# biddisco/hpx

Hardware: AMD Instinct MI355X
Metric: achieved GB/s (% HBM peak) for triad/reduce/scan/sort at 2^30, 1-8 MI355X (higher is better)
Workload: dtype f64+int64; 1 GPU; STREAM triad (f64) + transform_reduce (int64) + inclusive_scan (int64) per step; elements_per_gpu=1073741824, global_elements=1073741824, partitioning=partitioned_vector x1

## Files before the change

### hpx_amd/_lib.py

```python
from __future__ import annotations

import ctypes
import os
import threading

_HERE = os.path.dirname(os.path.abspath(__file__))
LIB_PATH = os.path.join(_HERE, "libhpxhip.so")

I32, U32, I64, U64, F32, F64 = range(6)
PLUS, MULTIPLIES, MIN, MAX, BIT_AND, BIT_OR, BIT_XOR = range(7)
U_IDENTITY, U_SCALE, U_ADD_SCALAR, U_AFFINE, U_NEGATE, U_ABS, U_SQUARE = range(7)
B_ADD, B_TRIAD, B_SUB, B_MUL, B_AXPY, B_MIN, B_MAX = range(7)
P_LT, P_LE, P_GT, P_GE, P_EQ, P_NE, P_NOT_LT, P_BITS = range(8)
H2H, H2D, D2H, D2D, DEFAULT = range(5)
GEN_IOTA, GEN_BITS, GEN_RANGE, GEN_UNIT = range(4)
(ALGO_REDUCE, ALGO_SCAN, ALGO_COPY_IF, ALGO_SORT, ALGO_SORT_BY_KEY, ALGO_MERGE, ALGO_MERGE_RUNS,
 ALGO_REDUCE_BY_KEY) = range(8)
STENCIL_MAX_FUSED = 16

SUCCESS = 0
ERROR_INVALID_ARGUMENT = 10001
ERROR_UNSUPPORTED = 10002
ERROR_DEVICE_TIMEOUT = 10003
ERROR_OUT_OF_MEMORY = 10004
# ... 84 lines not shown
    "hpxhip_stream_device": [_vp, ctypes.POINTER(_i)],
    "hpxhip_event_destroy": [_vp],
    "hpxhip_event_record": [_vp, _vp],
    "hpxhip_event_synchronize": [_vp],
    "hpxhip_event_query": [_vp],
    "hpxhip_event_elapsed_ms": [_vp, _vp, ctypes.POINTER(_f)],
    "hpxhip_stream_wait_event": [_vp, _vp],
    "hpxhip_malloc": [_i, ctypes.POINTER(_vp), _sz],
    "hpxhip_free": [_vp],
    "hpxhip_malloc_host": [ctypes.POINTER(_vp), _sz],
    "hpxhip_free_host": [_vp],
    "hpxhip_mem_info": [_i, ctypes.POINTER(_sz), ctypes.POINTER(_sz)],
    "hpxhip_memcpy_async": [_vp, _vp, _sz, _i, _vp],
    "hpxhip_memcpy_peer_async": [_vp, _i, _vp, _i, _sz, _vp],
    "hpxhip_memset_async": [_vp, _i, _sz, _vp],
    "hpxhip_scratch_bytes": [_i, _i, _i, _u64, ctypes.POINTER(_sz)],
    "hpxhip_stream_scratch": [_vp, _sz, ctypes.POINTER(_vp)],
    "hpxhip_device_error_word": [_vp, ctypes.POINTER(_vp)],
    "hpxhip_generate": [_i, _i, _u64, ctypes.c_int64, ctypes.c_int64, _vp, _u64, _vp],
    "hpxhip_generate_at": [_i, _i, _u64, _u64, ctypes.c_int64, ctypes.c_int64, _vp, _u64, _vp],
    "hpxhip_fill": [_i, _vp, _vp, _u64, _vp],
    "hpxhip_copy": [_i, _vp, _vp, _u64, _vp],
    "hpxhip_for_each": [_i, _i, _vp, _vp, _u64, _vp],
    "hpxhip_transform": [_i, _i, _i, _i, _vp, _vp, _vp, _u64, _vp],
    "hpxhip_transform_binary": [_i, _i, _i, _i, _vp, _vp, _vp, _vp, _u64, _vp],
    "hpxhip_transform_strided": [_i, _i, _i, _i, _vp, _vp, ctypes.c_int64, _vp, ctypes.c_int64, _u64, _vp],
    "hpxhip_transform_binary_strided": [_i, _i, _i, _i, _vp, _vp, ctypes.c_int64, _vp, ctypes.c_int64, _vp,
                                        ctypes.c_int64, _u64, _vp],
    "hpxhip_transform_reduce": [_i, _i, _i, _i, _vp, _vp, _vp, _u64, _vp, _vp, _vp, _sz],
    "hpxhip_transform_reduce_binary": [_i, _i, _i, _i, _vp, _vp, _vp, _vp, _u64, _vp, _vp, _vp, _sz],
    "hpxhip_fold": [_i, _i, _vp, _vp, _u64, _vp, _vp],
    "hpxhip_fold_exclusive": [_i, _i, _vp, _vp, _u64, _vp, _vp],
    "hpxhip_scan": [_i, _i, _i, _i, _vp, _vp, _vp, _vp, _vp, _u64, _vp, _vp, _sz],
    "hpxhip_copy_if": [_i, _i, _vp, _vp, _vp, _u64, _vp, _vp, _vp, _sz],
    "hpxhip_reduce_by_key": [_i, _i, _i, _vp, _vp, _vp, _vp, _u64, _vp, _vp, _vp, _sz],
    "hpxhip_sort": [_i, _vp, _u64, _i, _vp, _vp, _sz],
    "hpxhip_sort_by_key": [_i, _i, _vp, _vp, _u64, _i, _vp, _vp, _sz],
    "hpxhip_merge": [_i, _vp, _u64, _vp, _u64, _vp, _i, _vp, _vp, _sz],
    "hpxhip_merge_runs": [_i, _vp, _vp, _i, _vp, _i, _vp, _vp, _sz],
    "hpxhip_unsorted_pairs": [_i, _vp, _u64, _i, _vp, _vp],
    "hpxhip_sorted_bounds": [_i, _vp, _u64, _vp, _u64, _i, _i, _vp, _vp],
    "hpxhip_stencil_heat_step": [_vp, _vp, _u64, _vp, _vp, _d, _d, _d, _vp],
    "hpxhip_stencil_heat_run": [_vp, _vp, _u64, _u64, _d, _d, _d, _vp],
    "hpxhip_stencil_heat_steps": [_vp, _vp, _u64, _u64, _u64, _vp, _vp, _i, _d, _d, _d, _vp],
    "hpxhip_stencil_heat_run_fused": [_vp, _vp, _u64, _u64, _d, _d, _d, ctypes.POINTER(_i), _vp],
}

_lib = None
_lock = threading.Lock()


def _preload_torch():
    if os.environ.get("HPXHIP_NO_TORCH"):
        return
    try:
        import torch
    except Exception:
        pass


ABI_VERSION = 1


def load(path: str | None = None):
    global _lib
    with _lock:
# ... 53 lines not shown
```

### hpx_amd/csrc/scan.hip

```cpp
#include <cstdlib>

#include "internal.hpp"
#include <hpxhip/kernels/lookback.hpp>
#include <hpxhip/kernels/reduce_by_key_kernel.hpp>
#include <hpxhip/kernels/scan_kernel.hpp>

using namespace hpxhip;

namespace {

using namespace hpxhip::scan_detail;

constexpr size_t kSlotsOff = 256;

template <typename T, int ROUNDS, int THREADS = kThreads>
uint64_t ntiles_for(uint64_t n) {
    return (n + tile_elems<T, ROUNDS, THREADS>() - 1) / tile_elems<T, ROUNDS, THREADS>();
}

template <typename T, bool ALIGNED>
constexpr int threads_for() {
    return (ALIGNED && (std::is_integral_v<T> || sizeof(T) == 8) && rounds_for<T, ALIGNED>() == 16) ? 512 : kThreads;
}

template <typename T>
size_t carry_off(uint64_t n) {
    return align_up(kSlotsOff + ntiles_for<T, 8>(n) * tile_state<T>::bytes_per_tile(), 256);
}
template <typename T>
size_t scratch_total(uint64_t n) {
    return carry_off<T>(n) + 256;
}

template <typename T, bool INCL, bool ALIGNED, bool SHIFTED = false, typename Conv, typename Op>
int launch_scan(const T* in, T* out, uint64_t n, Conv conv, Op op, T init, const T* prefix_dev, char* ws,
                hipStream_t s) {
    static_assert(ALIGNED || !SHIFTED, "a shifted input needs the vector kernel");
    constexpr int R = rounds_for<T, ALIGNED>();
    constexpr int TH = threads_for<T, ALIGNED>();
    static_assert(tile_elems<T, R, TH>() >= tile_elems<T, 8>(), "scratch is sized for 1024 x 8-round tiles");
    const uint64_t ntiles = ntiles_for<T, R, TH>(n);
    HPXHIP_CHECK(hipMemsetAsync(ws, 0, align_up(kSlotsOff + ntiles * tile_state<T>::bytes_per_tile(), 256), s));
    scan_detail::scan_state<T> st{reinterpret_cast<uint64_t*>(ws + kSlotsOff), device_error_word(s)};
    hipLaunchKernelGGL((k_scan<T, Conv, Op, INCL, ALIGNED, R, TH, true, TH == kThreads ? 1 : 4, false, 1,
                               HPXHIP_TILE_DYN_ID, true, T, std::is_floating_point_v<T> && sizeof(T) == 8, true,
                               SHIFTED>),
                       dim3(static_cast<unsigned>(ntiles)), dim3(TH), 0, s, in, out, n, conv, op, init, prefix_dev,
                       reinterpret_cast<uint32_t*>(ws), st);
    HPXHIP_CHECK_LAUNCH();
    return 0;
}

template <typename T, bool INCL, typename Conv, typename Op>
__global__ void k_scan_head(const T* in, T* out, uint64_t h, Conv conv, Op op, T init, const T* prefix_dev,
                            T* carry) {
    if (threadIdx.x != 0 || blockIdx.x != 0) return;
    T acc = prefix_dev ? *prefix_dev : init;
    for (uint64_t i = 0; i < h; ++i) {
        const T x = conv(in[i]);
        if (INCL) {
            acc = op(acc, x);
            out[i] = acc;
        } else {
            out[i] = acc;
            acc = op(acc, x);
        }
    }
    *carry = acc;
}

template <typename T, bool INCL, typename Conv, typename Op>
int launch_scan_split(const T* in, T* out, uint64_t n, Conv conv, Op op, T init, const T* prefix_dev, char* ws,
                      hipStream_t s) {
    const uintptr_t ia = reinterpret_cast<uintptr_t>(in), oa = reinterpret_cast<uintptr_t>(out);
    if (ia % sizeof(T) != 0 || oa % sizeof(T) != 0) return -1;
    uint64_t h = head_to_align16(out, sizeof(T));
    const uintptr_t v = oa + h * sizeof(T);
    h += ((1024 - v % 1024) % 1024) / sizeof(T);
    if (n <= 4 * h + 1024) return -1;
    T* carry = reinterpret_cast<T*>(ws + carry_off<T>(n));
    hipLaunchKernelGGL((k_scan_head<T, INCL, Conv, Op>), dim3(1), dim3(64), 0, s, in, out, h, conv, op, init,
                       prefix_dev, carry);
    HPXHIP_CHECK_LAUNCH();
    if (ia % 16 == oa % 16) return launch_scan<T, INCL, true>(in + h, out + h, n - h, conv, op, init, carry, ws, s);
    return launch_scan<T, INCL, true, true>(in + h, out + h, n - h, conv, op, init, carry, ws, s);
}

template <typename T, typename F>
int with_scan_conv(int kind, const void* scalars, F&& f) {
    switch (kind) {
        case HPXHIP_U_IDENTITY:
        case HPXHIP_U_SCALE:
        case HPXHIP_U_SQUARE: break;
        default: return HPXHIP_ERROR_UNSUPPORTED;
    }
    return with_unary<T>(kind, scalars, [&](auto conv) -> int {
        using C = decltype(conv);
        if constexpr (std::is_same_v<C, unary_fn<HPXHIP_U_IDENTITY, T>> ||
                      std::is_same_v<C, unary_fn<HPXHIP_U_SCALE, T>> ||
                      std::is_same_v<C, unary_fn<HPXHIP_U_SQUARE, T>>)
            return f(conv);
        else
            return HPXHIP_ERROR_UNSUPPORTED;
    });
}

}

namespace hpxhip {
size_t scan_scratch_bytes(int dtype, uint64_t n) {
    return dtype_size(dtype) == 8 ? scratch_total<uint64_t>(n) : scratch_total<uint32_t>(n);
}
}

namespace {

namespace rbk = hpxhip::reduce_by_key_detail;

// ... 44 lines not shown
    return launch_reduce_by_key_ct<K, V, uint32_t>(kp, vp, ko, vo, n, f, count_dev, base, s);
}

template <typename F>
int with_key_class(int key_dtype, F&& f) {
    switch (key_dtype) {
        case HPXHIP_I32:
        case HPXHIP_U32: return f(tag<uint32_t>{});
        case HPXHIP_I64:
        case HPXHIP_U64: return f(tag<uint64_t>{});
        case HPXHIP_F32: return f(tag<float>{});
        case HPXHIP_F64: return f(tag<double>{});
        default: return HPXHIP_ERROR_INVALID_ARGUMENT;
    }
}

template <typename V, typename F>
int with_value_op(int op, F&& f) {
    if constexpr (std::is_integral_v<V> && std::is_signed_v<V>) {
        switch (op) {
            case HPXHIP_MIN: return f(op_min{});
            case HPXHIP_MAX: return f(op_max{});
            default: return HPXHIP_ERROR_INVALID_ARGUMENT;
        }
    } else {
        return with_binop<V>(op, f);
    }
}

__global__ void k_zero_u64(uint64_t* c) {
    if (threadIdx.x == 0 && blockIdx.x == 0) *c = 0;
}

}

namespace hpxhip {
size_t reduce_by_key_scratch_bytes(int key_dtype, int value_dtype, uint64_t n) {
    (void)key_dtype;
    return dtype_size(value_dtype) == 8 ? rbk_state_bytes<uint64_t, uint64_t>(n, true)
                                        : rbk_state_bytes<uint64_t, uint32_t>(n, true);
}
}

extern "C" int hpxhip_reduce_by_key(int key_dtype, int value_dtype, int op, const void* keys_in,
                                    const void* values_in, void* keys_out, void* values_out, uint64_t n,
                                    uint64_t* count_dev, hpxhip_stream stream, void* scratch, size_t scratch_bytes) {
    HPXHIP_ANNOTATE("hpxhip_reduce_by_key");
    if (!count_dev || (n && (!keys_in || !values_in || !keys_out || !values_out)))
        return HPXHIP_ERROR_INVALID_ARGUMENT;
    if (dtype_size(key_dtype) == 0 || dtype_size(value_dtype) == 0) return HPXHIP_ERROR_INVALID_ARGUMENT;
    if (op < HPXHIP_PLUS || op > HPXHIP_BIT_XOR) return HPXHIP_ERROR_INVALID_ARGUMENT;
    hipStream_t s = reinterpret_cast<hipStream_t>(stream);
    device_guard g(s);
    if (g.status) return g.status;
    if (n == 0) {
        hipLaunchKernelGGL(k_zero_u64, dim3(1), dim3(64), 0, s, count_dev);
        HPXHIP_CHECK_LAUNCH();
        return 0;
    }
    if (op != HPXHIP_MIN && op != HPXHIP_MAX) {
        if (value_dtype == HPXHIP_I32) value_dtype = HPXHIP_U32;
        if (value_dtype == HPXHIP_I64) value_dtype = HPXHIP_U64;
    }
    return with_key_class(key_dtype, [&](auto kt) -> int {
        using K = typename decltype(kt)::type;
        return with_dtype(value_dtype, [&](auto vt) -> int {
            using V = typename decltype(vt)::type;
            return with_value_op<V>(op, [&](auto o) -> int {
                return launch_reduce_by_key<K, V>(keys_in, values_in, keys_out, values_out, n, o, count_dev, s,
                                                  scratch, scratch_bytes);
            });
        });
    });
}

extern "C" int hpxhip_scan(int dtype, int op, int inclusive, int conv_kind, const void* conv_scalars,
                           const void* init, const void* prefix_dev, const void* in, void* out, uint64_t n,
                           hpxhip_stream stream, void* scratch, size_t scratch_bytes) {
    HPXHIP_ANNOTATE("hpxhip_scan");
    if (n == 0) return 0;
    if (!in || !out || (!init && !prefix_dev)) return HPXHIP_ERROR_INVALID_ARGUMENT;
    hipStream_t s = reinterpret_cast<hipStream_t>(stream);
    device_guard g(s);
    if (g.status) return g.status;
    return with_dtype(dtype, [&](auto t) -> int {
        using T = typename decltype(t)::type;
        T iv = T(0);
        if (init) __builtin_memcpy(&iv, init, sizeof(T));
        return with_binop<T>(op, [&](auto o) -> int {
            return with_scan_conv<T>(conv_kind, conv_scalars, [&](auto conv) -> int {
                void* ws = nullptr;
                int rc = resolve_scratch(s, scratch, scratch_bytes, scratch_total<T>(n), &ws);
                if (rc) return rc;
                char* base = static_cast<char*>(ws);
                const bool aligned = (reinterpret_cast<uintptr_t>(in) % 16 == 0) &&
                                     (reinterpret_cast<uintptr_t>(out) % 16 == 0);
                const T* pd = static_cast<const T*>(prefix_dev);
                const T* ip = static_cast<const T*>(in);
                T* op_ = static_cast<T*>(out);
                if (inclusive) {
                    if (aligned) return launch_scan<T, true, true>(ip, op_, n, conv, o, iv, pd, base, s);
                    const int r = launch_scan_split<T, true>(ip, op_, n, conv, o, iv, pd, base, s);
                    return r >= 0 ? r : launch_scan<T, true, false>(ip, op_, n, conv, o, iv, pd, base, s);
                }
                if (aligned) return launch_scan<T, false, true>(ip, op_, n, conv, o, iv, pd, base, s);
                const int r = launch_scan_split<T, false>(ip, op_, n, conv, o, iv, pd, base, s);
                return r >= 0 ? r : launch_scan<T, false, false>(ip, op_, n, conv, o, iv, pd, base, s);
            });
        });
    });
}
```

### hpx_amd/segmented.py

```python
from __future__ import annotations

import contextlib
import ctypes
import os

import numpy as np

from . import _lib as L
from . import functional as F
from .compute import dtype_code, np_dtype, target, vector


def partition_bounds(n: int, parts: int, k: int):
    part = -(-n // parts) if parts else 0
    b = min(n, k * part)
    return b, min(n, b + part)


def rank_partitions(k: int, p: int, r: int):
    c = -(-k // p) if p else 0
    a = min(k, r * c)
    return a, min(k, a + c)


# ... 217 lines not shown
            self.mem.put(h[0:c], send_left, nb, stream)
            self.mem.put(h[M:M + c], send_right, nb, stream)
            for w in dist.batch_isend_irecv(ring_halo_ops(dist, self.rank, self.size, h[0:c], h[M:M + c],
                                                           h[2 * M:2 * M + c], h[3 * M:3 * M + c])):
                w.wait()
            self.mem.get(recv_left, h[2 * M:2 * M + c], nb, stream)
            self.mem.get(recv_right, h[3 * M:3 * M + c], nb, stream)


class HipEngine:

    def __init__(self, tgt: target):
        self.tgt = tgt

    @property
    def stream(self):
        return self.tgt.stream

    def reduce_into(self, vec, lo, hi, op, conv, acc_dt, out_ptr, init=None):
        seed = _identity(op.kind, acc_dt) if init is None else init
        L.call("hpxhip_transform_reduce", vec.dtype, acc_dt, op.kind, conv.kind, L.scalars_buf(acc_dt, conv.scalars),
               L.scalar_buf(acc_dt, seed), ctypes.c_void_p(vec.data() + lo * vec.value_size), hi - lo,
               ctypes.c_void_p(out_ptr), self.stream, None, 0)

    def fold(self, dt, op, init, values_ptr, count, out_ptr):
        L.call("hpxhip_fold", dt, op.kind, L.scalar_buf(dt, init), ctypes.c_void_p(values_ptr), count,
               ctypes.c_void_p(out_ptr), self.stream)

    def scan(self, src, lo, hi, dst, dlo, op, conv, inclusive, prefix_ptr):
        dt = src.dtype
        L.call("hpxhip_scan", dt, op.kind, 1 if inclusive else 0, conv.kind, L.scalars_buf(dt, conv.scalars),
               L.scalar_buf(dt, 0), ctypes.c_void_p(prefix_ptr), ctypes.c_void_p(src.data() + lo * src.value_size),
               ctypes.c_void_p(dst.data() + dlo * dst.value_size), hi - lo, self.stream, None, 0)

    def transform(self, pol, pv, lo, hi, dst, dlo, f):
        from . import algorithms as A
        A.transform((pol or _par()).on(_exec(pv)), pv.local.begin() + lo, pv.local.begin() + hi, dst.begin() + dlo, f)

    def word(self, ptr, i, size=8):
        return ptr + size * int(i)

    def put(self, ptr, dt, value):
        L.call("hpxhip_fill", dt, L.scalar_buf(dt, value), ctypes.c_void_p(ptr), 1, self.stream)

    def read(self, ptr, dt):
        out = np.empty(1, np_dtype(dt))
        L.call("hpxhip_memcpy_async", out.ctypes.data_as(ctypes.c_void_p), ctypes.c_void_p(ptr), out.itemsize, L.D2H,
               self.stream)
        L.call("hpxhip_stream_synchronize", self.stream)
        return out[0].item()

    def sort(self, vec, lo, hi, descending):
        if hi - lo > 1:
            L.call("hpxhip_sort", vec.dtype, ctypes.c_void_p(vec.data() + lo * vec.value_size), hi - lo,
                   1 if descending else 0, self.stream, None, 0)

    def bounds(self, vec, lo, hi, values, upper, descending):
        values = np.ascontiguousarray(values, np_dtype(vec.dtype))
        m = values.size
        dv = vector.from_host(values, self.tgt)
        dout = vector(m, dtype=np.uint64, tgt=self.tgt)
        L.call("hpxhip_sorted_bounds", vec.dtype, ctypes.c_void_p(vec.data() + lo * vec.value_size), hi - lo,
               ctypes.c_void_p(dv.data()), m, 1 if upper else 0, 1 if descending else 0,
               ctypes.c_void_p(dout.data()), self.stream)
        out = dout.to_host()
        dv.free()
# ... 367 lines not shown
                return future.on_stream(eng.stream, thunk=lambda: _read_host(host, adt))
            return make_ready_future(eng.read(dev, adt))
        if isinstance(eng, HipEngine):
            from .algorithms import _read_host
            L.call("hpxhip_memcpy_async", ctypes.c_void_p(hslot), ctypes.c_void_p(dev), 8, L.D2H, eng.stream)
            L.call("hpxhip_stream_synchronize", eng.stream)
            return _read_host(hslot, adt)
        return eng.read(dev, adt)

    def reduce(self, pol, first, last, init=0, op=F.plus):
        return self.transform_reduce(pol, first, last, init, op, F.identity())

    def _scan(self, pol, first, last, dest, op, init, inclusive, conv):
        op = F.require(op, F.BinaryOp, "segmented scan")
        conv = F.require(conv, F.Unary, "segmented scan")
        pv, a, b = _range(first, last)
        pd, d0, _ = _range(dest, dest + (b - a))
        if pd.dtype != pv.dtype:
            raise TypeError("segmented scan: input and output element types must match")
        eng, comm = self.engine(pv), pv.comm
        plan = self._dest_plan(pv, a, b, pd, d0)
        direct, ia, ib, _, _, at = plan
        from .algorithms import _slots_for
        def carry_slot():
            return _slots_for(pv.tgt).next()[0] if isinstance(eng, HipEngine) else eng.scratch()
        lo0 = ia - pv.lo
        out, out0 = (pd.local, at) if direct else (eng.buffer(pd.local, ib - ia), 0)
        if pv.parts == 1:
            carry = carry_slot()
            send, recv = comm.slots(8)
            eng.fold(pv.dtype, op, init, recv, 0, carry)
            if ib > ia:
                eng.scan(pv.local, lo0, ib - pv.lo, out, out0, op, conv, inclusive, carry)
        else:
            recv, cmax = self._segment_totals(pv, a, b, op, conv, pv.dtype, eng, comm)
            j0, j1 = pv.my_segments()
            for i, j in enumerate(range(j0, j1)):
                s0, s1 = pv.segment_bounds(j)
                lo, hi = pv.local_range(max(s0, a), min(s1, b))
                if hi <= lo:
                    continue
                carry = carry_slot()
                eng.fold(pv.dtype, op, init, recv, comm.rank * cmax + i, carry)
                eng.scan(pv.local, lo, hi, out, out0 + (lo - lo0), op, conv, inclusive, carry)
        if not direct:
            self._finish_dest(eng, comm, plan, out, pd)
        return dest + (b - a)

    def inclusive_scan(self, pol, first, last, dest, op=F.plus, init=0):
        return self._scan(pol, first, last, dest, op, init, True, F.identity())

    def exclusive_scan(self, pol, first, last, dest, init, op=F.plus):
        return self._scan(pol, first, last, dest, op, init, False, F.identity())

    def transform_inclusive_scan(self, pol, first, last, dest, op, conv, init=0):
        return self._scan(pol, first, last, dest, op, init, True, conv)

    def transform_exclusive_scan(self, pol, first, last, dest, init, op, conv):
        return self._scan(pol, first, last, dest, op, init, False, conv)

    def sort(self, pol, first, last=None, comp=F.less):
        comp = F.require(comp, F.Compare, "segmented sort")
        pv, a, b = _range(first, last)
        if a != 0 or b != pv.n:
            raise ValueError("segmented sort sorts a whole partitioned_vector")
        eng, comm = self.engine(pv), pv.comm
# ... 270 lines not shown
```

### include/hpx/parallel/algorithms.hpp

```cpp
#pragma once

#include <hpx/compute/hip.hpp>
#include <hpx/compute/hip/concurrent_executor.hpp>
#include <hpx/compute/hip/default_executor.hpp>
#include <hpx/compute/hip/functional.hpp>
#include <hpx/parallel/detail/device_algorithms.hpp>
#include <hpx/parallel/detail/device_closures.hpp>
#include <hpx/parallel/execution.hpp>
#include <hpx/parallel/segmented_fwd.hpp>

#include <algorithm>
#include <array>
#include <cstring>
#include <functional>
#include <iterator>
#include <tuple>
#include <type_traits>
#include <vector>

namespace hpx { namespace parallel {
inline namespace v1 {

namespace detail {
namespace hip = hpx::compute::hip;
// ... 412 lines not shown
    if constexpr (tr::is_binop<Op> && tr::is_unary<Conv>) {
        T s[2] = {};
        tr::unary_t<Conv>::scalars(conv, s);
        check(hpxhip_transform_reduce(dt<TI>, dt<T>, tr::binop_t<Op>::kind, tr::unary_t<Conv>::kind, s, &init, first, n,
                                      out_dev, t.stream(), nullptr, 0),
              "transform_reduce");
    } else {
#if HPX_HAVE_HIP_DEVICE_CLOSURES
        dev::reduce<T, false>(t, first, static_cast<TI const*>(nullptr), n, init, op, conv, out_dev);
#else
        no_device_mapping<Op>("transform_reduce");
#endif
    }
}

template <typename V, typename Op, typename Conv, typename T>
void scan_into(hip::target const& t, V const* first, V* out, uint64_t n, Op const& op, Conv const& conv, T init,
               V const* prefix_dev, bool inclusive) {
    if constexpr (tr::is_binop<Op> && tr::is_unary<Conv>) {
        V s[2] = {};
        tr::unary_t<Conv>::scalars(conv, s);
        V iv = static_cast<V>(init);
        check(hpxhip_scan(dt<V>, tr::binop_t<Op>::kind, inclusive ? 1 : 0, tr::unary_t<Conv>::kind, s, &iv, prefix_dev,
                          first, out, n, t.stream(), nullptr, 0),
              inclusive ? "inclusive_scan" : "exclusive_scan");
    } else {
#if HPX_HAVE_HIP_DEVICE_CLOSURES
        if (prefix_dev)
            throw hpx::exception(HPXHIP_ERROR_UNSUPPORTED, "scan: a device prefix needs a built-in operator");
        dev::scan(t, first, out, n, op, conv, init, inclusive);
#else
        no_device_mapping<Op>(inclusive ? "inclusive_scan" : "exclusive_scan");
#endif
    }
}

template <typename T, typename P, typename It, typename Op, typename Conv>
result_t<P, T> reduce_impl(P&& p, It first, It last, T init, Op&& op, Conv&& conv) {
    if constexpr (is_seg<It>) {
        return segmented_detail::reduce<T>(std::forward<P>(p), first, last, init, std::forward<Op>(op),
                                           std::forward<Conv>(conv));
    } else {
    static_assert(is_dev<It>, "reduce: device iterators required");
    using TI = value_t<It>;
    auto const& t = target_of(p, first);
    auto slot = t.make_result_slot();
    reduce_into<T>(t, static_cast<TI const*>(first.device_ptr()), distance(first, last), init, op, conv, slot.device());
    fetch_slot(t, slot, sizeof(T), "reduce result");
    return finish_slot<T>(p, t, std::move(slot), load_value<T>{});
    }
}
}
namespace algo {

template <typename P, typename It, typename T, typename Op>
detail::result_t<P, T> reduce(P&& p, It first, It last, T init, Op&& op) {
    return detail::reduce_impl<T>(std::forward<P>(p), first, last, init, std::forward<Op>(op),
                                  hpx::compute::hip::functional::identity{});
}
template <typename P, typename It, typename T>
detail::result_t<P, T> reduce(P&& p, It first, It last, T init) {
    return reduce(std::forward<P>(p), first, last, init, std::plus<T>());
}
template <typename P, typename It>
detail::result_t<P, detail::value_t<It>> reduce(P&& p, It first, It last) {
    using T = detail::value_t<It>;
// ... 637 lines not shown
```

### include/hpx/parallel/segmented_algorithms.hpp

```cpp
#pragma once

#include <hpx/parallel/algorithms.hpp>
#include <hpx/parallel/segmented_fwd.hpp>

#include <algorithm>
#include <limits>
#include <vector>

namespace hpx { namespace parallel { inline namespace v1 { namespace segmented_detail {

namespace ex = hpx::parallel::execution;

template <typename P>
constexpr bool task_policy = execution::is_async_execution_policy<typename std::decay<P>::type>::value;

struct segment {
    std::size_t part, lo, hi;
};

template <typename PV>
std::vector<segment> segments_of(PV& pv, std::size_t a, std::size_t b) {
    std::vector<segment> s;
    if (a >= b) return s;
    for (std::size_t j = pv.partition_of(a); j < pv.get_num_partitions(); ++j) {
        auto const& p = pv.get_partition(j);
        if (p.first >= b) break;
        const std::size_t lo = std::max(a, p.first), hi = std::min(b, p.last);
        if (hi > lo) s.push_back(segment{j, lo - p.first, hi - p.first});
    }
    return s;
}

template <typename It>
std::size_t index_of(It const& it) {
    return it.index();
}

template <typename T, typename Op>
// ... 76 lines not shown
    }
    Out end = dest + (last - first);
    return finish<R, P>(std::move(fs), [last, end] { return R{last, end}; });
}

template <typename P, typename In1, typename In2, typename Out, typename F>
typename util::detail::algorithm_result<P, util::tagged_tuple<In1, In2, Out>>::type transform_binary(
    P&&, In1 first1, std::size_t n, In2 first2, Out dest, F&& f) {
    using R = util::tagged_tuple<In1, In2, Out>;
    auto& pv = first1.container();
    auto& p2 = first2.container();
    auto& pd = dest.container();
    require_same_layout(pv, index_of(first1), p2, index_of(first2), "segmented transform");
    require_same_layout(pv, index_of(first1), pd, index_of(dest), "segmented transform");
    using L1 = typename std::decay<decltype(pv.get_partition(0).data->begin())>::type;
    using L2 = typename std::decay<decltype(p2.get_partition(0).data->begin())>::type;
    using LO = typename std::decay<decltype(pd.get_partition(0).data->begin())>::type;
    std::vector<hpx::future<util::tagged_tuple<L1, L2, LO>>> fs;
    const std::size_t a = index_of(first1);
    for (auto const& s : segments_of(pv, a, a + n)) {
        auto& d1 = *pv.get_partition(s.part).data;
        auto& d2 = *p2.get_partition(s.part).data;
        auto& o = *pd.get_partition(s.part).data;
        fs.push_back(hpx::parallel::transform(ex::par(ex::task), d1.begin() + s.lo, d1.begin() + s.hi,
                                              d2.begin() + s.lo, o.begin() + s.lo, f));
    }
    const auto d = static_cast<std::ptrdiff_t>(n);
    In1 e1 = first1 + d;
    In2 e2 = first2 + d;
    Out eo = dest + d;
    return finish<R, P>(std::move(fs), [e1, e2, eo] { return R{e1, e2, eo}; });
}

template <typename V, typename PV, typename Op, typename Conv>
struct segment_totals {
    std::vector<segment> segs;
    compute::hip::target const* t0 = nullptr;
    compute::hip::detail::device_pool* pool0 = nullptr;
    compute::hip::detail::device_pool::block_ref blk{};
    std::vector<compute::hip::result_slot> slots;

    V* totals() const { return static_cast<V*>(blk.dev); }
    V* carries() const { return reinterpret_cast<V*>(static_cast<char*>(blk.dev) + 16 * ((segs.size() * sizeof(V) + 15) / 16)); }

    segment_totals(PV& pv, std::size_t a, std::size_t b, Op const& op, Conv const& conv) : segs(segments_of(pv, a, b)) {
        namespace hd = compute::hip::detail;
        if (segs.empty()) return;
        t0 = &pv.get_partition(segs[0].part).target;
        pool0 = &hd::device_pool::get(t0->device());
        const std::size_t nseg = segs.size();
        blk = pool0->acquire_block(16 * ((nseg * sizeof(V) + 15) / 16) + (nseg + 1) * sizeof(V));
        const V id = identity_of<V, typename std::decay<Op>::type>();
        for (std::size_t j = 0; j < nseg; ++j) {
            auto const& s = segs[j];
            auto& part = pv.get_partition(s.part);
            auto const& tj = part.target;
            slots.push_back(tj.make_result_slot());
            detail::reduce_into<V>(tj, part.data->data() + s.lo, s.hi - s.lo, id, op, conv, slots[j].device());
            copy_value(totals() + j, *t0, slots[j].device(), tj, tj.stream());
            hd::stream_after(t0->stream(), tj.stream());
        }
    }
    static void copy_value(void* dst, compute::hip::target const& dt, void const* src, compute::hip::target const& st,
                           hpxhip_stream s) {
        namespace hd = compute::hip::detail;
        if (dt.device() == st.device())
            hd::check(hpxhip_memcpy_async(dst, src, sizeof(V), HPXHIP_D2D, s), "segment value copy");
        else
            hd::check(hpxhip_memcpy_peer_async(dst, dt.device(), src, st.device(), sizeof(V), s),
                      "segment value peer copy");
    }
    void release_block_after(hpxhip_stream s) {
        auto* pool = pool0;
        auto b = blk;
        compute::hip::detail::on_stream_done(s, [pool, b] { pool->release_block(b); });
    }
};

template <typename T, typename P, typename It, typename Op, typename Conv>
typename util::detail::algorithm_result<P, T>::type reduce(P&& p, It first, It last, T init, Op&& op, Conv&& conv) {
    auto& pv = first.container();
    using PV = typename std::decay<decltype(pv)>::type;
    static_assert(compute::hip::traits::is_binop<Op>,
                  "segmented reduce: the segment-order combine runs on the device with a built-in operator");
    segment_totals<T, PV, Op, Conv> st(pv, index_of(first), index_of(last), op, conv);
    if (st.segs.empty()) {
        if constexpr (task_policy<P>) return hpx::make_ready_future(init);
        else return init;
    }
    auto const& t0 = *st.t0;
    auto slot = t0.make_result_slot();
    compute::hip::detail::check(hpxhip_fold(detail::dt<T>, compute::hip::traits::binop_t<Op>::kind, &init, st.totals(),
                                            st.segs.size(), slot.device(), t0.stream()),
                                "segmented reduce fold");
    detail::fetch_slot(t0, slot, sizeof(T), "segmented reduce result");
    st.release_block_after(t0.stream());
    for (std::size_t j = 0; j < st.segs.size(); ++j)
        pv.get_partition(st.segs[j].part).target.template async_result<void>([](unsigned char const*) {},
                                                                              std::move(st.slots[j]));
    return detail::finish_slot<T>(p, t0, std::move(slot), detail::load_value<T>{});
}

template <typename P, typename In, typename Out, typename Op, typename Conv, typename T>
typename util::detail::algorithm_result<P, Out>::type scan(P&&, In first, In last, Out dest, Op&& op, Conv&& conv,
                                                          T init, bool inclusive) {
    namespace hd = compute::hip::detail;
    auto& pv = first.container();
    auto& pd = dest.container();
    require_same_layout(pv, index_of(first), pd, index_of(dest), "segmented scan");
    using PV = typename std::decay<decltype(pv)>::type;
    using V = typename PV::value_type;
    static_assert(compute::hip::traits::is_binop<Op>,
                  "segmented scan: the carries are folded on the device with a built-in operator");
    Out end = dest + (last - first);
    segment_totals<V, PV, Op, Conv> st(pv, index_of(first), index_of(last), op, conv);
    if (st.segs.empty()) {
        if constexpr (task_policy<P>) return hpx::make_ready_future(end);
        else return end;
    }
    auto const& t0 = *st.t0;
    const V iv = static_cast<V>(init);
    hd::check(hpxhip_fold_exclusive(detail::dt<V>, compute::hip::traits::binop_t<Op>::kind, &iv, st.totals(),
                                    st.segs.size(), st.carries(), t0.stream()),
              "segmented scan carries");
    std::vector<hpx::future<void>> fs;
    for (std::size_t j = 0; j < st.segs.size(); ++j) {
        auto const& s = st.segs[j];
        auto& part = pv.get_partition(s.part);
        auto const& tj = part.target;
        V* carry = reinterpret_cast<V*>(static_cast<char*>(st.slots[j].device()) + 16);
        hd::stream_after(tj.stream(), t0.stream());
        st.copy_value(carry, tj, st.carries() + j, t0, tj.stream());
        auto& o = *pd.get_partition(s.part).data;
        detail::scan_into(tj, part.data->data() + s.lo, o.data() + s.lo, s.hi - s.lo, op, conv, iv, carry, inclusive);
        hd::stream_after(t0.stream(), tj.stream());
        fs.push_back(tj.template async_result<void>([](unsigned char const*) {}, std::move(st.slots[j])));
    }
    st.release_block_after(t0.stream());
    if constexpr (task_policy<P>) {
        return hpx::when_all(std::move(fs)).then([end](auto& all) {
            for (auto& f : all.get()) f.get();
            return end;
        });
    } else {
        for (auto& f : fs) f.get();
        return end;
    }
}

template <typename P, typename In, typename Out>
typename util::detail::algorithm_result<P, util::tagged_pair<In, Out>>::type copy(P&&, In first, In last,
                                                                                 Out dest) {
    using R = util::tagged_pair<In, Out>;
    const auto n = last - first;
// ... 44 lines not shown
```

### include/hpxhip.h

```cpp
#ifndef HPXHIP_H
#define HPXHIP_H

#include <stddef.h>
#include <stdint.h>

#ifdef __cplusplus
extern "C" {
#endif

#define HPXHIP_ABI_VERSION 1

enum hpxhip_status {
    HPXHIP_SUCCESS = 0,
    HPXHIP_ERROR_INVALID_ARGUMENT = 10001,
    HPXHIP_ERROR_UNSUPPORTED = 10002,
    HPXHIP_ERROR_DEVICE_TIMEOUT = 10003,
    HPXHIP_ERROR_OUT_OF_MEMORY = 10004,
    HPXHIP_ERROR_NOT_READY = 10005
};

enum hpxhip_dtype {
    HPXHIP_I32 = 0,
    HPXHIP_U32 = 1,
    HPXHIP_I64 = 2,
// ... 138 lines not shown
int hpxhip_copy(int dtype, const void* in, void* out, uint64_t n, hpxhip_stream stream);
int hpxhip_for_each(int dtype, int unary_kind, const void* scalars, void* data, uint64_t n,
                    hpxhip_stream stream);
int hpxhip_transform(int in_dtype, int compute_dtype, int out_dtype, int unary_kind,
                     const void* scalars, const void* in, void* out, uint64_t n,
                     hpxhip_stream stream);
int hpxhip_transform_binary(int in_dtype, int compute_dtype, int out_dtype, int binary_kind,
                            const void* scalars, const void* in1, const void* in2, void* out,
                            uint64_t n, hpxhip_stream stream);
int hpxhip_transform_strided(int in_dtype, int compute_dtype, int out_dtype, int unary_kind,
                             const void* scalars, const void* in, int64_t in_stride, void* out,
                             int64_t out_stride, uint64_t n, hpxhip_stream stream);
int hpxhip_transform_binary_strided(int in_dtype, int compute_dtype, int out_dtype, int binary_kind,
                                    const void* scalars, const void* in1, int64_t in1_stride,
                                    const void* in2, int64_t in2_stride, void* out,
                                    int64_t out_stride, uint64_t n, hpxhip_stream stream);

int hpxhip_transform_reduce(int in_dtype, int acc_dtype, int red_op, int conv_kind,
                            const void* conv_scalars, const void* init, const void* in,
                            uint64_t n, void* out_dev, hpxhip_stream stream, void* scratch,
                            size_t scratch_bytes);
int hpxhip_transform_reduce_binary(int in_dtype, int acc_dtype, int red_op, int binary_kind,
                                   const void* bin_scalars, const void* init, const void* in1,
                                   const void* in2, uint64_t n, void* out_dev,
                                   hpxhip_stream stream, void* scratch, size_t scratch_bytes);
int hpxhip_fold(int dtype, int op, const void* init, const void* values_dev, uint64_t count,
                void* out_dev, hpxhip_stream stream);
int hpxhip_fold_exclusive(int dtype, int op, const void* init, const void* values_dev, uint64_t count,
                          void* out_dev, hpxhip_stream stream);

int hpxhip_scan(int dtype, int op, int inclusive, int conv_kind, const void* conv_scalars,
                const void* init, const void* prefix_dev, const void* in, void* out,
                uint64_t n, hpxhip_stream stream, void* scratch, size_t scratch_bytes);

int hpxhip_copy_if(int dtype, int pred_kind, const void* pred_arg, const void* in, void* out,
                   uint64_t n, uint64_t* count_dev, hpxhip_stream stream, void* scratch,
                   size_t scratch_bytes);

int hpxhip_reduce_by_key(int key_dtype, int value_dtype, int op, const void* keys_in,
                         const void* values_in, void* keys_out, void* values_out, uint64_t n,
                         uint64_t* count_dev, hpxhip_stream stream, void* scratch,
                         size_t scratch_bytes);

int hpxhip_sort(int dtype, void* keys, uint64_t n, int descending, hpxhip_stream stream,
                void* scratch, size_t scratch_bytes);
int hpxhip_sort_by_key(int key_dtype, int value_dtype, void* keys, void* values, uint64_t n,
                       int descending, hpxhip_stream stream, void* scratch, size_t scratch_bytes);

int hpxhip_merge(int dtype, const void* in1, uint64_t n1, const void* in2, uint64_t n2, void* out,
                 int descending, hpxhip_stream stream, void* scratch, size_t scratch_bytes);
int hpxhip_merge_runs(int dtype, const void* in, const uint64_t* run_offsets, int nruns, void* out,
                      int descending, hpxhip_stream stream, void* scratch, size_t scratch_bytes);
int hpxhip_sorted_bounds(int dtype, const void* sorted, uint64_t n, const void* values_dev, uint64_t m,
                         int upper, int descending, uint64_t* out_dev, hpxhip_stream stream);

int hpxhip_unsorted_pairs(int dtype, const void* keys, uint64_t n, int descending, uint64_t* count_dev,
                          hpxhip_stream stream);

int hpxhip_stencil_heat_step(const double* cur, double* next, uint64_t n,
                             const double* left_halo_dev, const double* right_halo_dev,
                             double k, double dt, double dx, hpxhip_stream stream);
#define HPXHIP_STENCIL_MAX_FUSED 16
int hpxhip_stencil_heat_steps(const double* cur, double* next, uint64_t n, uint64_t out_lo, uint64_t out_hi,
                              const double* left_halo_dev, const double* right_halo_dev, int steps, double k,
                              double dt, double dx, hpxhip_stream stream);
int hpxhip_stencil_heat_run(double* u0, double* u1, uint64_t n, uint64_t nt, double k,
// ... 10 lines not shown
```

Measured before the change: 6808 GB/s.

## Chain segment scans on one device instead of precomputing segment totals

When every segment of a partitioned-vector scan lives on one device, each segment is scanned in sequence, and a small kernel emits that segment's total from the decoupled-lookback tile state to seed the next segment. This replaces the separate reduction pass over all segments, plus the carry fold, so the input is read once instead of twice. The cost is serialising the segments on the stream and one extra single-wave kernel per segment. The Python path gets the same treatment for single-rank HIP engines.

```diff
diff --git a/hpx_amd/_lib.py b/hpx_amd/_lib.py
--- a/hpx_amd/_lib.py
+++ b/hpx_amd/_lib.py
@@ -140,6 +140,8 @@
     "hpxhip_fold": [_i, _i, _vp, _vp, _u64, _vp, _vp],
     "hpxhip_fold_exclusive": [_i, _i, _vp, _vp, _u64, _vp, _vp],
     "hpxhip_scan": [_i, _i, _i, _i, _vp, _vp, _vp, _vp, _vp, _u64, _vp, _vp, _sz],
+    "hpxhip_scan_total": [_i, _i, _i, _i, _vp, _vp, _vp, _vp, _vp, _u64, _vp, _vp, _vp, _sz],
+    "hpxhip_scan_tile_elems": [_i, ctypes.POINTER(_u64)],
     "hpxhip_copy_if": [_i, _i, _vp, _vp, _vp, _u64, _vp, _vp, _vp, _sz],
     "hpxhip_reduce_by_key": [_i, _i, _i, _vp, _vp, _vp, _vp, _u64, _vp, _vp, _vp, _sz],
     "hpxhip_sort": [_i, _vp, _u64, _i, _vp, _vp, _sz],
diff --git a/hpx_amd/csrc/scan.hip b/hpx_amd/csrc/scan.hip
--- a/hpx_amd/csrc/scan.hip
+++ b/hpx_amd/csrc/scan.hip
@@ -32,9 +32,25 @@
     return carry_off<T>(n) + 256;
 }
 
+template <typename T, typename Op>
+__global__ __launch_bounds__(kWave) void k_scan_total(scan_detail::scan_state<T> st, uint64_t ntiles, Op op,
+                                                      T* total) {
+    const uint64_t tile = ntiles - 1;
+    uint32_t spins = 0;
+    T p = Op::template identity<T>(), agg = p;
+    bool ok = true;
+    if (tile == 0) ok = st.wait_slot(0, TILE_INCLUSIVE, &p, spins);
+    else p = st.exclusive_prefix_fixed(tile, op);
+    ok = st.wait_slot(tile, TILE_AGGREGATE, &agg, spins) && ok;
+    if (lane_id() != 0) return;
+    if (!ok && st.err)
+        __hip_atomic_store(st.err, HPXHIP_DEVERR_LOOKBACK_TIMEOUT, __ATOMIC_RELAXED, __HIP_MEMORY_SCOPE_AGENT);
+    *total = op(p, agg);
+}
+
 template <typename T, bool INCL, bool ALIGNED, bool SHIFTED = false, typename Conv, typename Op>
-int launch_scan(const T* in, T* out, uint64_t n, Conv conv, Op op, T init, const T* prefix_dev, char* ws,
-                hipStream_t s) {
+int launch_scan(const T* in, T* out, uint64_t n, Conv conv, Op op, T init, const T* prefix_dev, T* total_dev,
+                char* ws, hipStream_t s) {
     static_assert(ALIGNED || !SHIFTED, "a shifted input needs the vector kernel");
     constexpr int R = rounds_for<T, ALIGNED>();
     constexpr int TH = threads_for<T, ALIGNED>();
@@ -48,6 +64,10 @@
                        dim3(static_cast<unsigned>(ntiles)), dim3(TH), 0, s, in, out, n, conv, op, init, prefix_dev,
                        reinterpret_cast<uint32_t*>(ws), st);
     HPXHIP_CHECK_LAUNCH();
+    if (total_dev) {
+        hipLaunchKernelGGL((k_scan_total<T, Op>), dim3(1), dim3(kWave), 0, s, st, ntiles, op, total_dev);
+        HPXHIP_CHECK_LAUNCH();
+    }
     return 0;
 }
 
@@ -70,8 +90,8 @@
 }
 
 template <typename T, bool INCL, typename Conv, typename Op>
-int launch_scan_split(const T* in, T* out, uint64_t n, Conv conv, Op op, T init, const T* prefix_dev, char* ws,
-                      hipStream_t s) {
+int launch_scan_split(const T* in, T* out, uint64_t n, Conv conv, Op op, T init, const T* prefix_dev,
+                      T* total_dev, char* ws, hipStream_t s) {
     const uintptr_t ia = reinterpret_cast<uintptr_t>(in), oa = reinterpret_cast<uintptr_t>(out);
     if (ia % sizeof(T) != 0 || oa % sizeof(T) != 0) return -1;
     uint64_t h = head_to_align16(out, sizeof(T));
@@ -82,8 +102,9 @@
     hipLaunchKernelGGL((k_scan_head<T, INCL, Conv, Op>), dim3(1), dim3(64), 0, s, in, out, h, conv, op, init,
                        prefix_dev, carry);
     HPXHIP_CHECK_LAUNCH();
-    if (ia % 16 == oa % 16) return launch_scan<T, INCL, true>(in + h, out + h, n - h, conv, op, init, carry, ws, s);
-    return launch_scan<T, INCL, true, true>(in + h, out + h, n - h, conv, op, init, carry, ws, s);
+    if (ia % 16 == oa % 16)
+        return launch_scan<T, INCL, true>(in + h, out + h, n - h, conv, op, init, carry, total_dev, ws, s);
+    return launch_scan<T, INCL, true, true>(in + h, out + h, n - h, conv, op, init, carry, total_dev, ws, s);
 }
 
 template <typename T, typename F>
@@ -194,6 +215,11 @@
     if (threadIdx.x == 0 && blockIdx.x == 0) *c = 0;
 }
 
+template <typename T>
+__global__ void k_scan_total_empty(T init, const T* prefix_dev, T* total) {
+    if (threadIdx.x == 0 && blockIdx.x == 0) *total = prefix_dev ? *prefix_dev : init;
+}
+
 }
 
 namespace hpxhip {
@@ -236,12 +262,11 @@
     });
 }
 
-extern "C" int hpxhip_scan(int dtype, int op, int inclusive, int conv_kind, const void* conv_scalars,
-                           const void* init, const void* prefix_dev, const void* in, void* out, uint64_t n,
-                           hpxhip_stream stream, void* scratch, size_t scratch_bytes) {
-    HPXHIP_ANNOTATE("hpxhip_scan");
-    if (n == 0) return 0;
-    if (!in || !out || (!init && !prefix_dev)) return HPXHIP_ERROR_INVALID_ARGUMENT;
+static int scan_impl(int dtype, int op, int inclusive, int conv_kind, const void* conv_scalars, const void* init,
+                     const void* prefix_dev, const void* in, void* out, uint64_t n, void* total_dev,
+                     hpxhip_stream stream, void* scratch, size_t scratch_bytes) {
+    if (n == 0 && !total_dev) return 0;
+    if ((n && (!in || !out)) || (!init && !prefix_dev)) return HPXHIP_ERROR_INVALID_ARGUMENT;
     hipStream_t s = reinterpret_cast<hipStream_t>(stream);
     device_guard g(s);
     if (g.status) return g.status;
@@ -249,6 +274,13 @@
         using T = typename decltype(t)::type;
         T iv = T(0);
         if (init) __builtin_memcpy(&iv, init, sizeof(T));
+        const T* pd = static_cast<const T*>(prefix_dev);
+        T* td = static_cast<T*>(total_dev);
+        if (n == 0) {
+            hipLaunchKernelGGL(k_scan_total_empty<T>, dim3(1), dim3(64), 0, s, iv, pd, td);
+            HPXHIP_CHECK_LAUNCH();
+            return 0;
+        }
         return with_binop<T>(op, [&](auto o) -> int {
             return with_scan_conv<T>(conv_kind, conv_scalars, [&](auto conv) -> int {
                 void* ws = nullptr;
@@ -257,18 +289,43 @@
                 char* base = static_cast<char*>(ws);
                 const bool aligned = (reinterpret_cast<uintptr_t>(in) % 16 == 0) &&
                                      (reinterpret_cast<uintptr_t>(out) % 16 == 0);
-                const T* pd = static_cast<const T*>(prefix_dev);
                 const T* ip = static_cast<const T*>(in);
                 T* op_ = static_cast<T*>(out);
                 if (inclusive) {
-                    if (aligned) return launch_scan<T, true, true>(ip, op_, n, conv, o, iv, pd, base, s);
-                    const int r = launch_scan_split<T, true>(ip, op_, n, conv, o, iv, pd, base, s);
-                    return r >= 0 ? r : launch_scan<T, true, false>(ip, op_, n, conv, o, iv, pd, base, s);
+                    if (aligned) return launch_scan<T, true, true>(ip, op_, n, conv, o, iv, pd, td, base, s);
+                    const int r = launch_scan_split<T, true>(ip, op_, n, conv, o, iv, pd, td, base, s);
+                    return r >= 0 ? r : launch_scan<T, true, false>(ip, op_, n, conv, o, iv, pd, td, base, s);
                 }
-                if (aligned) return launch_scan<T, false, true>(ip, op_, n, conv, o, iv, pd, base, s);
-                const int r = launch_scan_split<T, false>(ip, op_, n, conv, o, iv, pd, base, s);
-                return r >= 0 ? r : launch_scan<T, false, false>(ip, op_, n, conv, o, iv, pd, base, s);
+                if (aligned) return launch_scan<T, false, true>(ip, op_, n, conv, o, iv, pd, td, base, s);
+                const int r = launch_scan_split<T, false>(ip, op_, n, conv, o, iv, pd, td, base, s);
+                return r >= 0 ? r : launch_scan<T, false, false>(ip, op_, n, conv, o, iv, pd, td, base, s);
             });
         });
     });
 }
+
+extern "C" int hpxhip_scan(int dtype, int op, int inclusive, int conv_kind, const void* conv_scalars,
+                           const void* init, const void* prefix_dev, const void* in, void* out, uint64_t n,
+                           hpxhip_stream stream, void* scratch, size_t scratch_bytes) {
+    HPXHIP_ANNOTATE("hpxhip_scan");
+    return scan_impl(dtype, op, inclusive, conv_kind, conv_scalars, init, prefix_dev, in, out, n, nullptr, stream,
+                     scratch, scratch_bytes);
+}
+
+extern "C" int hpxhip_scan_tile_elems(int dtype, uint64_t* tile_elems) {
+    if (!tile_elems) return HPXHIP_ERROR_INVALID_ARGUMENT;
+    return with_dtype(dtype, [&](auto t) -> int {
+        using T = typename decltype(t)::type;
+        *tile_elems = scan_detail::tile_elems<T, rounds_for<T, true>(), threads_for<T, true>()>();
+        return 0;
+    });
+}
+
+extern "C" int hpxhip_scan_total(int dtype, int op, int inclusive, int conv_kind, const void* conv_scalars,
+                                 const void* init, const void* prefix_dev, const void* in, void* out, uint64_t n,
+                                 void* total_dev, hpxhip_stream stream, void* scratch, size_t scratch_bytes) {
+    HPXHIP_ANNOTATE("hpxhip_scan_total");
+    if (!total_dev || total_dev == prefix_dev) return HPXHIP_ERROR_INVALID_ARGUMENT;
+    return scan_impl(dtype, op, inclusive, conv_kind, conv_scalars, init, prefix_dev, in, out, n, total_dev, stream,
+                     scratch, scratch_bytes);
+}
diff --git a/hpx_amd/segmented.py b/hpx_amd/segmented.py
--- a/hpx_amd/segmented.py
+++ b/hpx_amd/segmented.py
@@ -273,6 +273,14 @@
         L.call("hpxhip_scan", dt, op.kind, 1 if inclusive else 0, conv.kind, L.scalars_buf(dt, conv.scalars),
                L.scalar_buf(dt, 0), ctypes.c_void_p(prefix_ptr), ctypes.c_void_p(src.data() + lo * src.value_size),
                ctypes.c_void_p(dst.data() + dlo * dst.value_size), hi - lo, self.stream, None, 0)
+
+    def scan_total(self, src, lo, hi, dst, dlo, op, conv, inclusive, init, prefix_ptr, total_ptr):
+        dt = src.dtype
+        L.call("hpxhip_scan_total", dt, op.kind, 1 if inclusive else 0, conv.kind,
+               L.scalars_buf(dt, conv.scalars), L.scalar_buf(dt, init),
+               ctypes.c_void_p(prefix_ptr) if prefix_ptr is not None else None,
+               ctypes.c_void_p(src.data() + lo * src.value_size), ctypes.c_void_p(dst.data() + dlo * dst.value_size),
+               hi - lo, ctypes.c_void_p(total_ptr), self.stream, None, 0)
 
     def transform(self, pol, pv, lo, hi, dst, dlo, f):
         from . import algorithms as A
@@ -706,6 +714,17 @@
             eng.fold(pv.dtype, op, init, recv, 0, carry)
             if ib > ia:
                 eng.scan(pv.local, lo0, ib - pv.lo, out, out0, op, conv, inclusive, carry)
+        elif isinstance(eng, HipEngine) and comm.size == 1:
+            prev = None
+            j0, j1 = pv.my_segments()
+            for j in range(j0, j1):
+                s0, s1 = pv.segment_bounds(j)
+                lo, hi = pv.local_range(max(s0, a), min(s1, b))
+                if hi <= lo:
+                    continue
+                total = carry_slot()
+                eng.scan_total(pv.local, lo, hi, out, out0 + (lo - lo0), op, conv, inclusive, init, prev, total)
+                prev = total
         else:
             recv, cmax = self._segment_totals(pv, a, b, op, conv, pv.dtype, eng, comm)
             j0, j1 = pv.my_segments()
diff --git a/include/hpx/parallel/algorithms.hpp b/include/hpx/parallel/algorithms.hpp
--- a/include/hpx/parallel/algorithms.hpp
+++ b/include/hpx/parallel/algorithms.hpp
@@ -468,6 +468,21 @@
 #else
         no_device_mapping<Op>(inclusive ? "inclusive_scan" : "exclusive_scan");
 #endif
+    }
+}
+
+template <typename V, typename Op, typename Conv, typename T>
+void scan_total_into(hip::target const& t, V const* first, V* out, uint64_t n, Op const& op, Conv const& conv, T init,
+                     V const* prefix_dev, V* total_dev, bool inclusive) {
+    if constexpr (tr::is_binop<Op> && tr::is_unary<Conv>) {
+        V s[2] = {};
+        tr::unary_t<Conv>::scalars(conv, s);
+        V iv = static_cast<V>(init);
+        check(hpxhip_scan_total(dt<V>, tr::binop_t<Op>::kind, inclusive ? 1 : 0, tr::unary_t<Conv>::kind, s, &iv,
+                                prefix_dev, first, out, n, total_dev, t.stream(), nullptr, 0),
+              inclusive ? "inclusive_scan" : "exclusive_scan");
+    } else {
+        throw hpx::exception(HPXHIP_ERROR_UNSUPPORTED, "scan: a device total needs a built-in operator");
     }
 }
 
diff --git a/include/hpx/parallel/segmented_algorithms.hpp b/include/hpx/parallel/segmented_algorithms.hpp
--- a/include/hpx/parallel/segmented_algorithms.hpp
+++ b/include/hpx/parallel/segmented_algorithms.hpp
@@ -4,6 +4,7 @@
 #include <hpx/parallel/segmented_fwd.hpp>
 
 #include <algorithm>
+#include <atomic>
 #include <limits>
 #include <vector>
 
@@ -146,6 +147,11 @@
     return finish<R, P>(std::move(fs), [e1, e2, eo] { return R{e1, e2, eo}; });
 }
 
+inline std::atomic<unsigned long>& segment_totals_passes() {
+    static std::atomic<unsigned long> n{0};
+    return n;
+}
+
 template <typename V, typename PV, typename Op, typename Conv>
 struct segment_totals {
     std::vector<segment> segs;
@@ -160,6 +166,7 @@
     segment_totals(PV& pv, std::size_t a, std::size_t b, Op const& op, Conv const& conv) : segs(segments_of(pv, a, b)) {
         namespace hd = compute::hip::detail;
         if (segs.empty()) return;
+        segment_totals_passes().fetch_add(1);
         t0 = &pv.get_partition(segs[0].part).target;
         pool0 = &hd::device_pool::get(t0->device());
         const std::size_t nseg = segs.size();
@@ -215,6 +222,50 @@
     return detail::finish_slot<T>(p, t0, std::move(slot), detail::load_value<T>{});
 }
 
+template <typename PV>
+bool on_one_device(PV& pv, std::vector<segment> const& segs) {
+    for (auto const& s : segs)
+        if (pv.get_partition(s.part).target.device() != pv.get_partition(segs[0].part).target.device()) return false;
+    return true;
+}
+
+template <typename P, typename PV, typename PD, typename Out, typename Op, typename Conv, typename V>
+typename util::detail::algorithm_result<P, Out>::type scan_chained(PV& pv, PD& pd, std::vector<segment> const& segs,
+                                                                  Out end, Op const& op, Conv const& conv, V iv,
+                                                                  bool inclusive) {
+    namespace hd = compute::hip::detail;
+    std::vector<hpx::future<void>> fs;
+    compute::hip::result_slot prev;
+    for (std::size_t j = 0; j < segs.size(); ++j) {
+        auto const& s = segs[j];
+        auto& part = pv.get_partition(s.part);
+        auto const& tj = part.target;
+        auto& o = *pd.get_partition(s.part).data;
+        V const* carry = prev ? static_cast<V const*>(prev.device()) : nullptr;
+        if (j > 0) hd::stream_after(tj.stream(), pv.get_partition(segs[j - 1].part).target.stream());
+        compute::hip::result_slot total;
+        if (j + 1 < segs.size()) {
+            total = tj.make_result_slot();
+            detail::scan_total_into(tj, part.data->data() + s.lo, o.data() + s.lo, s.hi - s.lo, op, conv, iv, carry,
+                                    static_cast<V*>(total.device()), inclusive);
+        } else {
+            detail::scan_into(tj, part.data->data() + s.lo, o.data() + s.lo, s.hi - s.lo, op, conv, iv, carry,
+                              inclusive);
+        }
+        fs.push_back(tj.template async_result<void>([](unsigned char const*) {}, std::move(prev)));
+        prev = std::move(total);
+    }
+    if constexpr (task_policy<P>) {
+        return hpx::when_all(std::move(fs)).then([end](auto& all) {
+            for (auto& f : all.get()) f.get();
+            return end;
+        });
+    } else {
+        for (auto& f : fs) f.get();
+        return end;
+    }
+}
+
 template <typename P, typename In, typename Out, typename Op, typename Conv, typename T>
 typename util::detail::algorithm_result<P, Out>::type scan(P&&, In first, In last, Out dest, Op&& op, Conv&& conv,
                                                           T init, bool inclusive) {
@@ -227,13 +278,17 @@
     static_assert(compute::hip::traits::is_binop<Op>,
                   "segmented scan: the carries are folded on the device with a built-in operator");
     Out end = dest + (last - first);
+    const V iv = static_cast<V>(init);
+    {
+        const std::vector<segment> segs = segments_of(pv, index_of(first), index_of(last));
+        if (segs.empty()) {
+            if constexpr (task_policy<P>) return hpx::make_ready_future(end);
+            else return end;
+        }
+        if (on_one_device(pv, segs)) return scan_chained<P>(pv, pd, segs, end, op, conv, iv, inclusive);
+    }
     segment_totals<V, PV, Op, Conv> st(pv, index_of(first), index_of(last), op, conv);
-    if (st.segs.empty()) {
-        if constexpr (task_policy<P>) return hpx::make_ready_future(end);
-        else return end;
-    }
     auto const& t0 = *st.t0;
-    const V iv = static_cast<V>(init);
     hd::check(hpxhip_fold_exclusive(detail::dt<V>, compute::hip::traits::binop_t<Op>::kind, &iv, st.totals(),
                                     st.segs.size(), st.carries(), t0.stream()),
               "segmented scan carries");
diff --git a/include/hpxhip.h b/include/hpxhip.h
--- a/include/hpxhip.h
+++ b/include/hpxhip.h
@@ -194,6 +194,11 @@
 int hpxhip_scan(int dtype, int op, int inclusive, int conv_kind, const void* conv_scalars,
                 const void* init, const void* prefix_dev, const void* in, void* out,
                 uint64_t n, hpxhip_stream stream, void* scratch, size_t scratch_bytes);
+int hpxhip_scan_total(int dtype, int op, int inclusive, int conv_kind, const void* conv_scalars,
+                      const void* init, const void* prefix_dev, const void* in, void* out,
+                      uint64_t n, void* total_dev, hpxhip_stream stream, void* scratch,
+                      size_t scratch_bytes);
+int hpxhip_scan_tile_elems(int dtype, uint64_t* tile_elems);
 
 int hpxhip_copy_if(int dtype, int pred_kind, const void* pred_arg, const void* in, void* out,
                    uint64_t n, uint64_t* count_dev, hpxhip_stream stream, void* scratch,
```

Result: no change. 6807 GB/s (-0.0%).
